# icdm-adteam/MoCoPCI

Measured on AMD Instinct MI355X. Metric: interpolated frames/sec, higher is better.
Workload: dtype f32 (fused MLP layers: fp32 products as 6 bf16-MFMA partials of an exact 3-way split, fp32 accumulate; index paths exact f32)

## Files before the change

### mocopci_amd/csrc/cross.hip

```cpp
#include "common.h"
#include "cross_tile.h"

#ifdef MCP_CROSS_DIAG
__device__ unsigned long long g_cross_diag[8];
#define CROSS_STAMP(slot)                                                                            \
    do {                                                                                             \
        unsigned long long t_;                                                                       \
        __builtin_amdgcn_sched_barrier(0);                                                           \
        asm volatile("s_memtime %0\n\ts_waitcnt lgkmcnt(0)" : "=s"(t_)::"memory");                   \
        __builtin_amdgcn_sched_barrier(0);                                                           \
        if (blockIdx.x == 0 && blockIdx.y == 0 && threadIdx.x == 0) g_cross_diag[slot] += t_ - t_prev; \
        t_prev = t_;                                                                                 \
    } while (0)
#else
#define CROSS_STAMP(slot)
#endif

namespace {

constexpr int MAX_MAPPED_BATCH = 1024;

template <int CTRL>
__device__ __forceinline__ float dppf(float v) {
    return __uint_as_float(mcp_dpp<CTRL>(__float_as_uint(v)));
}
#define MCP_MAX_DPP(dst, src0, src1, CTRL)                                                                              \
    asm("s_nop 1\n\tv_max_f32_dpp %0, %1, %2 " CTRL : "+v"(dst) : "v"(src0), "v"(src1))

__device__ __forceinline__ float scatter_max(const f32x16 &acc, int lane) {
    float v8[8], v4[4], v2[2];
#pragma unroll
    for (int r = 0; r < 8; ++r) {
        const auto sw = __builtin_amdgcn_permlane16_swap(__float_as_uint(acc[r]), __float_as_uint(acc[r + 8]), false, false);
        const float a = __uint_as_float(sw[0]), b = __uint_as_float(sw[1]);
        asm("v_max_f32 %0, %1, %2" : "=v"(v8[r]) : "v"(a), "v"(b));
    }
#pragma unroll
    for (int r = 0; r < 4; ++r) {
        float d = v8[r + 4];
        MCP_MAX_DPP(d, v8[r], v8[r], "row_ror:8 row_mask:0xf bank_mask:0x3");
        MCP_MAX_DPP(d, v8[r + 4], d, "row_ror:8 row_mask:0xf bank_mask:0xc");
        v4[r] = d;
    }
#pragma unroll
    for (int r = 0; r < 2; ++r) {
        float d = v4[r + 2];
        MCP_MAX_DPP(d, v4[r], v4[r], "row_half_mirror row_mask:0xf bank_mask:0x5");
        MCP_MAX_DPP(d, v4[r + 2], d, "row_half_mirror row_mask:0xf bank_mask:0xa");
        v2[r] = d;
    }
    const bool b1 = (lane & 2) != 0;
    float keep = b1 ? v2[1] : v2[0];
    const float send = b1 ? v2[0] : v2[1];
    MCP_MAX_DPP(keep, send, keep, "quad_perm:[2,3,0,1] row_mask:0xf bank_mask:0xf");
    MCP_MAX_DPP(keep, keep, keep, "quad_perm:[1,0,3,2] row_mask:0xf bank_mask:0xf");
    return keep;
}
__device__ __forceinline__ int scatter_reg(int lane) { return ((lane >> 4) & 1) * 8 + ((lane >> 3) & 1) * 4 + ((lane >> 2) & 1) * 2 + ((lane >> 1) & 1); }

template <int D>
__global__ __launch_bounds__(256) void cross_pack_kernel(const float *__restrict__ wpos, const float *__restrict__ bpos,
                                                         const float *__restrict__ wmlp, const float *__restrict__ bmlp,
                                                         float *__restrict__ packed) {
    using L = CrossLds<D>;
    for (int e = blockIdx.x * 256 + threadIdx.x; e < L::FLOATS; e += gridDim.x * 256) {
        float v;
        if (e < L::OFF_POS) continue;
        else if (e < L::OFF_B) {
            const int f = e - L::OFF_POS, lane = f & 63, s = (f >> 6) & 1, t = f >> 7;
            const int row = 32 * t + (lane & 31), c = 2 * s + (lane >> 5);
            v = c < 3 ? wpos[row * 3 + c] : bpos[row];
        } else {
            const int f = e - L::OFF_B, r = f & 15, h = (f >> 4) & 1, t = f >> 5;
            v = bmlp[32 * t + mcp_chan_of(r, h)];
        }
        packed[e] = v;
    }
    mcp_split_weights(reinterpret_cast<uint4 *>(packed + L::OFF_W), wmlp, D, L::T, blockIdx.x * 256 + threadIdx.x, gridDim.x * 256);
}

template <int D>
struct CrossShape {
    static constexpr int NW = D == 128 ? 8 : 4;
    static constexpr int WG_PER_CU = D == 64 ? 3 : 1;
    static constexpr int GRID = D == 64 ? 768 : 256;
};

template <int D, int SPLIT>
__global__ __launch_bounds__(64 * CrossShape<D>::NW, CrossShape<D>::WG_PER_CU) void cross_kernel(long long total, int n1, int n2, const float *__restrict__ xyz1,
                                                           const float *__restrict__ xyz2, const float *__restrict__ points1,
                                                           const float *__restrict__ points2, const int *__restrict__ idx,
                                                           const int *__restrict__ idx2, const int *__restrict__ bmap, int shared,
                                                           const float *__restrict__ packed, float *__restrict__ out) {
    using L = CrossLds<D>;
    constexpr int T = L::T;
    constexpr int WAVES = CrossShape<D>::NW;
    constexpr int TO = T / SPLIT;
    constexpr int WH = L::W_FLOATS / SPLIT, SMALL = L::POS_FLOATS + L::B_FLOATS;
    extern __shared__ __attribute__((aligned(16))) float lds[];
    const int tid = threadIdx.x, split = blockIdx.y;
    static_assert(WH % 4 == 0 && SMALL % 4 == 0, "LDS image is copied as float4");
    for (int e = tid; e < WH / 4; e += 64 * WAVES)
        reinterpret_cast<float4 *>(lds)[e] = reinterpret_cast<const float4 *>(packed + L::OFF_W + (size_t)split * WH)[e];
    for (int e = tid; e < SMALL / 4; e += 64 * WAVES)
        reinterpret_cast<float4 *>(lds + WH)[e] = reinterpret_cast<const float4 *>(packed + L::OFF_POS)[e];
    if (bmap) {
        const int nb = (int)(total / n1);
        for (int e = tid; e < nb; e += 64 * WAVES) reinterpret_cast<int *>(lds + WH + SMALL + WAVES * D)[e] = bmap[e];
    }
    __syncthreads();

    const int lane = tid & 63, wave = tid >> 6, h = lane >> 5, col = lane & 31;
    const float *lpos = lds + WH, *lbias = lds + WH + L::POS_FLOATS;
    float *row1_lds = lds + WH + SMALL + wave * D;
    const int *bmap_lds = reinterpret_cast<const int *>(lds + WH + SMALL + WAVES * D);

#ifndef MCP_NO_XCD_MAP
    const bool by_xcd = gridDim.x >= 8 && (gridDim.x & 7) == 0;
#else
    const bool by_xcd = false;
#endif
    const long long chunk = by_xcd ? (total + 7) / 8 : total;
    const long long stride = (long long)(by_xcd ? gridDim.x >> 3 : gridDim.x) * WAVES;
    const long long limit = by_xcd ? min(total, ((long long)(blockIdx.x & 7) + 1) * chunk) : total;
    long long p = by_xcd ? (long long)(blockIdx.x & 7) * chunk + (long long)(blockIdx.x >> 3) * WAVES + wave : (long long)blockIdx.x * WAVES + wave;
    float q2x = 0.f, q2y = 0.f, q2z = 0.f, p1x = 0.f, p1y = 0.f, p1z = 0.f;
    float4 r1 = make_float4(0.f, 0.f, 0.f, 0.f);
    float4 rg[T][4];
    auto mapped = [&](int bb, int flag) -> long long { return (bmap && (shared & flag)) ? (long long)bmap_lds[bb] : (long long)bb; };
    struct Pos { int bb, off; };
    const int stride_b = (int)(stride / n1), stride_o = (int)(stride % n1);
    auto advance = [&](Pos q) {
        q.bb += stride_b;
        q.off += stride_o;
        if (q.off >= n1) { q.off -= n1; ++q.bb; }
        return q;
    };
    auto fetch = [&](long long pp, Pos q, int id) {
        const float *q2 = xyz2 + ((long long)q.bb * n2 + id) * 3;
        q2x = q2[0]; q2y = q2[1]; q2z = q2[2];
        p1x = xyz1[pp * 3 + 0]; p1y = xyz1[pp * 3 + 1]; p1z = xyz1[pp * 3 + 2];
        const float4 *row2 = reinterpret_cast<const float4 *>(points2 + (mapped(q.bb, 2) * n2 + id) * D);
        const float4 *row1 = reinterpret_cast<const float4 *>(points1 + (mapped(q.bb, 1) * n1 + q.off) * D);
        r1 = row1[lane < D / 4 ? lane : 0];
#pragma unroll
        for (int t = 0; t < T; ++t)
#pragma unroll
            for (int g = 0; g < 4; ++g) rg[t][g] = row2[(32 * t + 8 * g + 4 * h) >> 2];
    };
    auto nbr = [&](long long pp, Pos q) { return cross_nbr(idx, idx2, pp, [&] { return mapped(q.bb, 4) * n1 + q.off; }, col); };
    long long pn = p + stride;
    Pos qp{(int)(p / n1), (int)(p % n1)};
    Pos qn = advance(qp), qnn = advance(qn);
    int idn = 0;
    if (p < limit) {
        fetch(p, qp, nbr(p, qp));
        if (pn < limit) idn = nbr(pn, qn);
    }
#ifdef MCP_CROSS_DIAG
    unsigned long long t_prev = 0;
    CROSS_STAMP(7);
#endif
    for (; p < limit; p = pn, pn += stride) {
        CROSS_STAMP(0);
        McpSplit3 xs[2 * T];
        const float in0 = h ? q2y - p1y : q2x - p1x, in1 = h ? 1.0f : q2z - p1z;
        if (lane < D / 4) reinterpret_cast<float4 *>(row1_lds)[lane] = r1;
        __builtin_amdgcn_wave_barrier();
#pragma unroll
        for (int t = 0; t < T; ++t) {
            f32x16 acc;
#pragma unroll
            for (int g = 0; g < 4; ++g) {
                const float4 a = reinterpret_cast<const float4 *>(row1_lds)[(32 * t + 8 * g + 4 * h) >> 2];
                acc[4 * g + 0] = a.x; acc[4 * g + 1] = a.y; acc[4 * g + 2] = a.z; acc[4 * g + 3] = a.w;
            }
            acc = __builtin_amdgcn_mfma_f32_32x32x2f32(lpos[(t * 2 + 0) * 64 + lane], in0, acc, 0, 0, 0);
            acc = __builtin_amdgcn_mfma_f32_32x32x2f32(lpos[(t * 2 + 1) * 64 + lane], in1, acc, 0, 0, 0);
#pragma unroll
            for (int g = 0; g < 4; ++g) {
                acc[4 * g + 0] = leaky(acc[4 * g + 0] + rg[t][g].x);
                acc[4 * g + 1] = leaky(acc[4 * g + 1] + rg[t][g].y);
                acc[4 * g + 2] = leaky(acc[4 * g + 2] + rg[t][g].z);
                acc[4 * g + 3] = leaky(acc[4 * g + 3] + rg[t][g].w);
            }
            xs[2 * t + 0] = mcp_split_kstep(acc, 0);
            xs[2 * t + 1] = mcp_split_kstep(acc, 1);
        }
        __builtin_amdgcn_wave_barrier();
        CROSS_STAMP(1);
        if (pn < limit) {
            fetch(pn, qn, idn);
            if (pn + stride < limit) idn = nbr(pn + stride, qnn);
        }
        qn = qnn;
        qnn = advance(qnn);
        CROSS_STAMP(2);
#pragma unroll 1
        for (int tl = 0; tl < TO; ++tl) {
            const int t = TO * split + tl;
            f32x16 acc;
#pragma unroll
            for (int r = 0; r < 16; ++r) acc[r] = lbias[(t * 2 + h) * 16 + r];
            acc = mcp_tile_split<2 * T>(reinterpret_cast<const uint4 *>(lds) + (size_t)tl * (2 * T) * 3 * 64 + lane, xs, acc);
            CROSS_STAMP(3);
            const float m = leaky(scatter_max(acc, lane));
            if ((lane & 1) == 0) out[p * D + 32 * t + mcp_chan_of(scatter_reg(lane), h)] = m;
            CROSS_STAMP(4);
        }
    }
}

__global__ __launch_bounds__(64 * X256_WAVES, 1) void cross256_stream_kernel(long long total, int n1, int n2, const float *__restrict__ xyz1,
                                                                          const float *__restrict__ xyz2, const float *__restrict__ points1,
                                                                          const float *__restrict__ points2, const int *__restrict__ idx,
                                                                          const int *__restrict__ idx2, const int *__restrict__ bmap, int shared,
                                                                          const float *__restrict__ packed, float *__restrict__ out) {
    using L = CrossLds<256>;
    constexpr int D = 256, T = X256_T, WAVES = X256_WAVES, SMALL = L::POS_FLOATS + L::B_FLOATS;
    extern __shared__ __attribute__((aligned(16))) float lds[];
    uint4 *wbuf = reinterpret_cast<uint4 *>(lds);
    float *small = lds + 2 * X256_TILE_U4 * 4;
    float *row1_all = small + SMALL;
    int *bmap_lds = reinterpret_cast<int *>(row1_all + WAVES * D);
    const int tid = threadIdx.x, lane = tid & 63, wave = tid >> 6, h = lane >> 5, col = lane & 31;
    const uint4 *wimg = reinterpret_cast<const uint4 *>(packed + L::OFF_W);
    for (int e = tid; e < SMALL / 4; e += 64 * WAVES) reinterpret_cast<float4 *>(small)[e] = reinterpret_cast<const float4 *>(packed + L::OFF_POS)[e];
    if (bmap) {
        const int nb = (int)(total / n1);
        for (int e = tid; e < nb; e += 64 * WAVES) bmap_lds[e] = bmap[e];
    }
    for (int e = tid; e < X256_TILE_U4; e += 64 * WAVES) wbuf[e] = wimg[e];
    __syncthreads();
    const float *lpos = small, *lbias = small + L::POS_FLOATS;
    float *row1_lds = row1_all + wave * D;
    auto mapped = [&](int bb, int flag) -> long long { return (bmap && (shared & flag)) ? (long long)bmap_lds[bb] : (long long)bb; };

    const long long per_round = (long long)gridDim.x * WAVES;
    const long long first = (long long)blockIdx.x * WAVES;
    const int rounds = first < total ? (int)((total - first + per_round - 1) / per_round) : 0;
    int cur = 0;
    for (int g = 0; g < rounds; ++g) {
        const long long pw = first + (long long)g * per_round + wave;
        const bool live = pw < total;
        const long long p = live ? pw : total - 1;
        const int bb = (int)(p / n1), off = (int)(p - (long long)bb * n1);
        int id;
        if (!idx2) {
            id = idx[p * KNB + col];
        } else {
            const long long ps = mapped(bb, 4) * n1 + off;
            id = col >= 16 ? idx2[p * 16 + col - 16] : idx[ps * 16 + col];
        }
        const float *q2 = xyz2 + ((long long)bb * n2 + id) * 3;
        const float dx = q2[0] - xyz1[p * 3 + 0], dy = q2[1] - xyz1[p * 3 + 1], dz = q2[2] - xyz1[p * 3 + 2];
        const float in0 = h ? dy : dx, in1 = h ? 1.0f : dz;
        const float4 *row2 = reinterpret_cast<const float4 *>(points2 + (mapped(bb, 2) * n2 + id) * D);
        const float4 *row1 = reinterpret_cast<const float4 *>(points1 + (mapped(bb, 1) * n1 + off) * D);
        reinterpret_cast<float4 *>(row1_lds)[lane] = row1[lane];
        __builtin_amdgcn_wave_barrier();
        McpSplit3 xs[2 * T];
#pragma unroll
        for (int t = 0; t < T; ++t) {
            f32x16 acc;
            float4 rg[4];
#pragma unroll
            for (int gq = 0; gq < 4; ++gq) {
                const float4 a = reinterpret_cast<const float4 *>(row1_lds)[(32 * t + 8 * gq + 4 * h) >> 2];
                rg[gq] = row2[(32 * t + 8 * gq + 4 * h) >> 2];
                acc[4 * gq + 0] = a.x; acc[4 * gq + 1] = a.y; acc[4 * gq + 2] = a.z; acc[4 * gq + 3] = a.w;
            }
            acc = __builtin_amdgcn_mfma_f32_32x32x2f32(lpos[(t * 2 + 0) * 64 + lane], in0, acc, 0, 0, 0);
            acc = __builtin_amdgcn_mfma_f32_32x32x2f32(lpos[(t * 2 + 1) * 64 + lane], in1, acc, 0, 0, 0);
#pragma unroll
            for (int gq = 0; gq < 4; ++gq) {
                acc[4 * gq + 0] = leaky(acc[4 * gq + 0] + rg[gq].x);
                acc[4 * gq + 1] = leaky(acc[4 * gq + 1] + rg[gq].y);
                acc[4 * gq + 2] = leaky(acc[4 * gq + 2] + rg[gq].z);
                acc[4 * gq + 3] = leaky(acc[4 * gq + 3] + rg[gq].w);
            }
            xs[2 * t + 0] = mcp_split_kstep(acc, 0);
            xs[2 * t + 1] = mcp_split_kstep(acc, 1);
        }
        __builtin_amdgcn_wave_barrier();
#pragma unroll 1
        for (int t = 0; t < T; ++t) {
            const bool more = t + 1 < T || g + 1 < rounds;
            const uint4 *nsrc = wimg + (size_t)((t + 1) & (T - 1)) * X256_TILE_U4 + tid;
            uint4 nx[X256_TILE_U4 / (64 * X256_WAVES)];
#pragma unroll
            for (int i = 0; i < X256_TILE_U4 / (64 * WAVES); ++i) nx[i] = more ? nsrc[i * 64 * WAVES] : make_uint4(0u, 0u, 0u, 0u);
            f32x16 acc;
#pragma unroll
            for (int r = 0; r < 16; ++r) acc[r] = lbias[(t * 2 + h) * 16 + r];
            acc = mcp_tile_split<2 * T>(wbuf + (size_t)cur * X256_TILE_U4 + lane, xs, acc);
            const float m = leaky(scatter_max(acc, lane));
            if (live && (lane & 1) == 0) out[p * D + 32 * t + mcp_chan_of(scatter_reg(lane), h)] = m;
            uint4 *ndst = wbuf + (size_t)(cur ^ 1) * X256_TILE_U4 + tid;
#pragma unroll
            for (int i = 0; i < X256_TILE_U4 / (64 * WAVES); ++i) ndst[i * 64 * WAVES] = nx[i];
            __syncthreads();
            cur ^= 1;
        }
    }
}

int launch_cross256(long long total, int n1, int n2, const float *xyz1, const float *xyz2, const float *points1, const float *points2, const int *idx,
                    const int *idx2, const int *bmap, int shared, const float *packed, float *out, hipStream_t s) {
    const size_t lds = (size_t)(X256_LDS_FLOATS + (bmap ? MAX_MAPPED_BATCH : 0)) * sizeof(float);
    if (const int rc = mcp_allow_lds<cross256_stream_kernel>()) return rc;
    const long long want = (total + X256_WAVES - 1) / X256_WAVES;
    const unsigned grid = (unsigned)max(1LL, min(want, 256LL));
    hipLaunchKernelGGL(cross256_stream_kernel, dim3(grid), dim3(64 * X256_WAVES), lds, s, total, n1, n2, xyz1, xyz2, points1, points2, idx, idx2, bmap, shared,
                       packed, out);
    return mcp_launch_status();
}

template <int D, int SPLIT>
int launch_cross(long long total, int n1, int n2, const float *xyz1, const float *xyz2, const float *points1, const float *points2,
                 const int *idx, const int *idx2, const int *bmap, int shared, const float *packed, float *out, hipStream_t s) {
    using L = CrossLds<D>;
    constexpr int WAVES = CrossShape<D>::NW;
    const size_t lds = (L::W_FLOATS / SPLIT + L::POS_FLOATS + L::B_FLOATS + WAVES * D + (bmap ? MAX_MAPPED_BATCH : 0)) * sizeof(float);
    constexpr auto kern = cross_kernel<D, SPLIT>;
    if (const int rc = mcp_allow_lds<kern>()) return rc;
    const long long want = (total + WAVES * 8 - 1) / (WAVES * 8);
    const unsigned grid = (unsigned)max(1LL, min(want, (long long)(CrossShape<D>::GRID / SPLIT)));
    hipLaunchKernelGGL(kern, dim3(grid, SPLIT), dim3(64 * WAVES), lds, s, total, n1, n2, xyz1, xyz2, points1, points2, idx, idx2, bmap, shared, packed, out);
    return mcp_launch_status();
}

}

MCP_EXPORT int mcp_cross_packed_floats(int d) {
    return d == 64 ? CrossLds<64>::FLOATS : d == 128 ? CrossLds<128>::FLOATS : d == 256 ? CrossLds<256>::FLOATS : 0;
}

MCP_EXPORT int mcp_cross_pack(int d, const float *wpos, const float *bpos, const float *wmlp, const float *bmlp, float *packed,
                              mcp_stream_t stream) {
    MCP_CHECK_ARGS(wpos && bpos && wmlp && bmlp && packed);
    if (d != 64 && d != 128 && d != 256) return MCP_ERR_UNSUPPORTED;
    if (((uintptr_t)packed) & 15) return MCP_ERR_BAD_ARG;
    hipStream_t s = (hipStream_t)stream;
    if (d == 64) hipLaunchKernelGGL(cross_pack_kernel<64>, dim3(16), dim3(256), 0, s, wpos, bpos, wmlp, bmlp, packed);
    else if (d == 128) hipLaunchKernelGGL(cross_pack_kernel<128>, dim3(64), dim3(256), 0, s, wpos, bpos, wmlp, bmlp, packed);
    else hipLaunchKernelGGL(cross_pack_kernel<256>, dim3(256), dim3(256), 0, s, wpos, bpos, wmlp, bmlp, packed);
    return mcp_launch_status();
}

MCP_EXPORT int mcp_cross_volume(int b, int n1, int n2, int d, int k, const float *xyz1, const float *xyz2, const float *points1,
                                const float *points2, const int *idx, const int *idx2, const int *bmap, int shared, const float *packed, float *out,
                                mcp_stream_t stream) {
    MCP_CHECK_ARGS(b > 0 && n1 > 0 && n2 > 0 && xyz1 && xyz2 && points1 && points2 && idx && packed && out);
    if (k != KNB || (d != 64 && d != 128 && d != 256)) return MCP_ERR_UNSUPPORTED;
    if ((((uintptr_t)points1) | ((uintptr_t)points2) | ((uintptr_t)out) | ((uintptr_t)packed)) & 15) return MCP_ERR_BAD_ARG;
    if (bmap && b > MAX_MAPPED_BATCH) return MCP_ERR_UNSUPPORTED;
    hipStream_t s = (hipStream_t)stream;
    const long long total = (long long)b * n1;
    mcp_prof_begin(MCP_KERNEL_CROSS, s);
    const int rc = d == 64    ? launch_cross<64, 1>(total, n1, n2, xyz1, xyz2, points1, points2, idx, idx2, bmap, shared, packed, out, s)
                   : d == 128 ? launch_cross<128, 1>(total, n1, n2, xyz1, xyz2, points1, points2, idx, idx2, bmap, shared, packed, out, s)
                              : launch_cross256(total, n1, n2, xyz1, xyz2, points1, points2, idx, idx2, bmap, shared, packed, out, s);
    mcp_prof_end(MCP_KERNEL_CROSS, s);
    return rc;
}

#ifdef MCP_CROSS_DIAG
MCP_EXPORT int mcp_cross_diag_read(unsigned long long *out8) {
    hipError_t e = hipMemcpyFromSymbol(out8, HIP_SYMBOL(g_cross_diag), sizeof(unsigned long long) * 8);
    unsigned long long z[8] = {0};
    (void)hipMemcpyToSymbol(HIP_SYMBOL(g_cross_diag), z, sizeof(z));
    return (int)e;
}
#endif
```

Before: 3669.

## Interleave layer-1 split work into layer-2 k-steps for D=128 cross kernel

For D=128 (by default), the cross kernel switches from a tile-major loop to a k-step-major schedule. The next tile's layer-1 MFMAs, leaky activation and 3-way bf16 split are interleaved as fill work inside the layer-2 MFMA k-steps, and the weight fragments for the next step are software-prefetched. The intent is to hide VALU split and activation work and LDS latency behind the MFMA pipeline, and to keep fewer split registers live. The cost is more accumulator registers (TO accumulators at once), more complex code, and possible register pressure or spills. The diagnostic timers also move to per-thread slot accumulation.

```diff
diff --git a/mocopci_amd/csrc/cross.hip b/mocopci_amd/csrc/cross.hip
--- a/mocopci_amd/csrc/cross.hip
+++ b/mocopci_amd/csrc/cross.hip
@@ -1,3 +1,4 @@
+#include <utility>
 #include "common.h"
 #include "cross_tile.h"
 
@@ -9,7 +10,7 @@
         __builtin_amdgcn_sched_barrier(0);                                                           \
         asm volatile("s_memtime %0\n\ts_waitcnt lgkmcnt(0)" : "=s"(t_)::"memory");                   \
         __builtin_amdgcn_sched_barrier(0);                                                           \
-        if (blockIdx.x == 0 && blockIdx.y == 0 && threadIdx.x == 0) g_cross_diag[slot] += t_ - t_prev; \
+        t_slot[slot] += t_ - t_prev;                                                                 \
         t_prev = t_;                                                                                 \
     } while (0)
 #else
@@ -84,7 +85,46 @@
     static constexpr int NW = D == 128 ? 8 : 4;
     static constexpr int WG_PER_CU = D == 64 ? 3 : 1;
     static constexpr int GRID = D == 64 ? 768 : 256;
+#if defined(MCP_CROSS_TILE_MAJOR)
+    static constexpr bool KSTEP_MAJOR = false;
+#elif defined(MCP_CROSS_KSTEP_MAJOR_64)
+    static constexpr bool KSTEP_MAJOR = true;
+#else
+    static constexpr bool KSTEP_MAJOR = D == 128;
+#endif
 };
+
+__device__ __forceinline__ void x0_pair(f32x16 &a, const float4 *rg, int i) {
+    const float4 g = rg[i >> 1];
+    a[2 * i + 0] = leaky(a[2 * i + 0] + ((i & 1) ? g.z : g.x));
+    a[2 * i + 1] = leaky(a[2 * i + 1] + ((i & 1) ? g.w : g.y));
+}
+__device__ __forceinline__ void split_pair(const f32x16 &a, int i, McpSplit3 *xs) {
+    const float v0 = a[2 * i], v1 = a[2 * i + 1];
+    const float r0 = v0 - __uint_as_float(mcp_top16(v0)), r1 = v1 - __uint_as_float(mcp_top16(v1));
+    const float s0 = r0 - __uint_as_float(mcp_top16(r0)), s1 = r1 - __uint_as_float(mcp_top16(r1));
+    const uint32_t d1 = mcp_pack_hi(v0, v1), d2 = mcp_pack_hi(r0, r1), d3 = mcp_pack_hi(s0, s1);
+    McpSplit3 &o = xs[i >> 2];
+    switch (i & 3) {
+        case 0: o.p1.x = d1; o.p2.x = d2; o.p3.x = d3; break;
+        case 1: o.p1.y = d1; o.p2.y = d2; o.p3.y = d3; break;
+        case 2: o.p1.z = d1; o.p2.z = d2; o.p3.z = d3; break;
+        default: o.p1.w = d1; o.p2.w = d2; o.p3.w = d3; break;
+    }
+}
+constexpr int NF_X0_PAIR = 6, NF_SPLIT_PAIR = 11;
+
+struct CrossFill { int l0, l1, s0, s1; };
+template <class F, int... I>
+__device__ __forceinline__ void cross_static_for_(F &&f, std::integer_sequence<int, I...>) { (f(std::integral_constant<int, I>{}), ...); }
+template <int N, class F>
+__device__ __forceinline__ void cross_static_for(F &&f) { cross_static_for_(f, std::make_integer_sequence<int, N>{}); }
+template <int NK>
+__device__ __forceinline__ constexpr CrossFill cross_fill(int j) {
+    if (NK == 4) return CrossFill{4 + j, 5 + j, 2 * j, 2 * j + 2};
+    if (j >= 3) return CrossFill{j, j + 1, j, j + 1};
+    return j == 0 ? CrossFill{0, 0, 0, 0} : j == 1 ? CrossFill{0, 2, 0, 1} : CrossFill{2, 3, 1, 3};
+}
 
 template <int D, int SPLIT>
 __global__ __launch_bounds__(64 * CrossShape<D>::NW, CrossShape<D>::WG_PER_CU) void cross_kernel(long long total, int n1, int n2, const float *__restrict__ xyz1,
@@ -148,21 +188,139 @@
 #pragma unroll
             for (int g = 0; g < 4; ++g) rg[t][g] = row2[(32 * t + 8 * g + 4 * h) >> 2];
     };
+    const int *bmap_any = bmap ? bmap_lds : reinterpret_cast<const int *>(lds);
+    auto mapped_sel = [&](int bb, int flag) -> long long {
+        const bool use = bmap && (shared & flag);
+        const int m = bmap_any[use ? bb : 0];
+        return use ? (long long)m : (long long)bb;
+    };
+    auto fetch_head = [&](long long pp, Pos q, int id) {
+        const float *q2 = xyz2 + ((long long)q.bb * n2 + id) * 3;
+        q2x = q2[0]; q2y = q2[1]; q2z = q2[2];
+        p1x = xyz1[pp * 3 + 0]; p1y = xyz1[pp * 3 + 1]; p1z = xyz1[pp * 3 + 2];
+        const float4 *row1 = reinterpret_cast<const float4 *>(points1 + (mapped_sel(q.bb, 1) * n1 + q.off) * D);
+        r1 = row1[lane < D / 4 ? lane : 0];
+    };
+    auto row2_of = [&](Pos q, int id) { return reinterpret_cast<const float4 *>(points2 + (mapped_sel(q.bb, 2) * n2 + id) * D); };
+    auto nbr_sel = [&](long long pp, int bb, int off) {
+        const long long ps = mapped_sel(bb, 4) * n1 + off;
+        const bool two = idx2 != nullptr, second = two && col >= 16;
+        const int *list = second ? idx2 : idx;
+        const long long row = two && !second ? ps : pp;
+        const long long at16 = row * 16 + (col & 15), at32 = row * KNB + col;
+        return list[two ? at16 : at32];
+    };
     auto nbr = [&](long long pp, Pos q) { return cross_nbr(idx, idx2, pp, [&] { return mapped(q.bb, 4) * n1 + q.off; }, col); };
     long long pn = p + stride;
     Pos qp{(int)(p / n1), (int)(p % n1)};
     Pos qn = advance(qp), qnn = advance(qn);
     int idn = 0;
+    [[maybe_unused]] int idc = 0;
+    [[maybe_unused]] Pos qc = qp;
     if (p < limit) {
-        fetch(p, qp, nbr(p, qp));
+        idc = nbr(p, qp);
+        fetch(p, qp, idc);
         if (pn < limit) idn = nbr(pn, qn);
     }
 #ifdef MCP_CROSS_DIAG
-    unsigned long long t_prev = 0;
+    unsigned long long t_prev = 0, t_slot[8] = {0, 0, 0, 0, 0, 0, 0, 0};
     CROSS_STAMP(7);
 #endif
     for (; p < limit; p = pn, pn += stride) {
         CROSS_STAMP(0);
+      if constexpr (CrossShape<D>::KSTEP_MAJOR) {
+        static_assert(SPLIT == 1 && (T == 2 || T == 4), "cross_fill's batches are laid out for 4 or 8 k-steps per block");
+        constexpr int NK = 2 * TO;
+        const float in0 = h ? q2y - p1y : q2x - p1x, in1 = h ? 1.0f : q2z - p1z;
+        if (lane < D / 4) reinterpret_cast<float4 *>(row1_lds)[lane] = r1;
+        __builtin_amdgcn_wave_barrier();
+        auto layer1_begin = [&](int t) {
+            f32x16 a;
+#pragma unroll
+            for (int g = 0; g < 4; ++g) {
+                const float4 v = reinterpret_cast<const float4 *>(row1_lds)[(32 * t + 8 * g + 4 * h) >> 2];
+                a[4 * g + 0] = v.x; a[4 * g + 1] = v.y; a[4 * g + 2] = v.z; a[4 * g + 3] = v.w;
+            }
+            a = __builtin_amdgcn_mfma_f32_32x32x2f32(lpos[(t * 2 + 0) * 64 + lane], in0, a, 0, 0, 0);
+            return __builtin_amdgcn_mfma_f32_32x32x2f32(lpos[(t * 2 + 1) * 64 + lane], in1, a, 0, 0, 0);
+        };
+        f32x16 xb[2];
+        McpSplit3 xs[2][2];
+        constexpr bool EARLY1 = NK == 4;
+        xb[0] = layer1_begin(0);
+        if constexpr (EARLY1) xb[1] = layer1_begin(1);
+        if constexpr (T == 2) __builtin_amdgcn_wave_barrier();
+#pragma unroll
+        for (int i = 0; i < 8; ++i) {
+            x0_pair(xb[0], rg[0], i);
+            split_pair(xb[0], i, xs[0]);
+        }
+        if constexpr (NK == 4) {
+#pragma unroll
+            for (int i = 0; i < 4; ++i) x0_pair(xb[1], rg[1], i);
+        }
+        __builtin_amdgcn_sched_barrier(0);
+        CROSS_STAMP(1);
+        const bool more = pn < limit;
+        idc = more ? idn : idc;
+        qc = more ? qn : qc;
+        const float4 *row2n = row2_of(qc, idc);
+        fetch_head(more ? pn : p, qc, idc);
+        const bool more2 = pn + stride < limit;
+        idn = nbr_sel(more2 ? pn + stride : more ? pn : p, more2 ? qnn.bb : qc.bb, more2 ? qnn.off : qc.off);
+#pragma unroll
+        for (int g = 0; g < 4; ++g) rg[0][g] = row2n[(8 * g + 4 * h) >> 2];
+        f32x16 acc[TO];
+#pragma unroll
+        for (int tl = 0; tl < TO; ++tl)
+#pragma unroll
+            for (int r = 0; r < 16; ++r) acc[tl][r] = lbias[((TO * split + tl) * 2 + h) * 16 + r];
+        const uint4 *wl = reinterpret_cast<const uint4 *>(lds) + lane;
+        uint4 w1 = wl[0], w2 = wl[64], w3 = wl[128];
+        cross_static_for<T>([&](auto tc) {
+            constexpr int t = decltype(tc)::value;
+            if constexpr ((t >= 1 || !EARLY1) && t + 1 < T) {
+                xb[(t + 1) & 1] = layer1_begin(t + 1);
+                if constexpr (t + 2 == T) __builtin_amdgcn_wave_barrier();
+            }
+            cross_static_for<NK>([&](auto jc) {
+                constexpr int j = decltype(jc)::value, tl = j % TO, ks = j / TO;
+                uint4 n1 = w1, n2 = w2, n3 = w3;
+                if constexpr (t * NK + j + 1 < T * NK) {
+                    constexpr int jn = (j + 1) % NK, tn = t + (j + 1) / NK;
+                    const uint4 *nx = wl + (size_t)((jn % TO) * 2 * T + 2 * tn + jn / TO) * 3 * 64;
+                    n1 = nx[0]; n2 = nx[64]; n3 = nx[128];
+                }
+                const McpSplit3 &x = xs[t & 1][ks];
+                if constexpr (t + 1 < T) {
+                    constexpr CrossFill f = cross_fill<NK>(j);
+                    constexpr int nf = NF_X0_PAIR * (f.l1 - f.l0) + NF_SPLIT_PAIR * (f.s1 - f.s0), u = t + 1;
+                    acc[tl] = mcp_kstep_fill<nf>(w1, w2, w3, x, acc[tl], [&] {
+#pragma unroll
+                        for (int i = f.l0; i < f.l1; ++i) x0_pair(xb[u & 1], rg[u], i);
+#pragma unroll
+                        for (int i = f.s0; i < f.s1; ++i) split_pair(xb[u & 1], i, xs[u & 1]);
+                    });
+                } else {
+                    acc[tl] = mcp_kstep_fill<0>(w1, w2, w3, x, acc[tl], [] {});
+                }
+                w1 = n1; w2 = n2; w3 = n3;
+            });
+            CROSS_STAMP(2 + t);
+            if constexpr (t + 1 < T) {
+#pragma unroll
+                for (int g = 0; g < 4; ++g) rg[t + 1][g] = row2n[(32 * (t + 1) + 8 * g + 4 * h) >> 2];
+            }
+        });
+#pragma unroll
+        for (int tl = 0; tl < TO; ++tl) {
+            const float m = leaky(scatter_max(acc[tl], lane));
+            if ((lane & 1) == 0) out[p * D + 32 * (TO * split + tl) + mcp_chan_of(scatter_reg(lane), h)] = m;
+        }
+        CROSS_STAMP(6);
+        qn = qnn;
+        qnn = advance(qnn);
+      } else {
         McpSplit3 xs[2 * T];
         const float in0 = h ? q2y - p1y : q2x - p1x, in1 = h ? 1.0f : q2z - p1z;
         if (lane < D / 4) reinterpret_cast<float4 *>(row1_lds)[lane] = r1;
@@ -188,14 +346,13 @@
             xs[2 * t + 1] = mcp_split_kstep(acc, 1);
         }
         __builtin_amdgcn_wave_barrier();
-        CROSS_STAMP(1);
         if (pn < limit) {
             fetch(pn, qn, idn);
             if (pn + stride < limit) idn = nbr(pn + stride, qnn);
         }
         qn = qnn;
         qnn = advance(qnn);
-        CROSS_STAMP(2);
+        CROSS_STAMP(1);
 #pragma unroll 1
         for (int tl = 0; tl < TO; ++tl) {
             const int t = TO * split + tl;
@@ -203,12 +360,17 @@
 #pragma unroll
             for (int r = 0; r < 16; ++r) acc[r] = lbias[(t * 2 + h) * 16 + r];
             acc = mcp_tile_split<2 * T>(reinterpret_cast<const uint4 *>(lds) + (size_t)tl * (2 * T) * 3 * 64 + lane, xs, acc);
-            CROSS_STAMP(3);
+            CROSS_STAMP(2);
             const float m = leaky(scatter_max(acc, lane));
             if ((lane & 1) == 0) out[p * D + 32 * t + mcp_chan_of(scatter_reg(lane), h)] = m;
-            CROSS_STAMP(4);
-        }
-    }
+            CROSS_STAMP(6);
+        }
+      }
+    }
+#ifdef MCP_CROSS_DIAG
+    if (blockIdx.x == 0 && blockIdx.y == 0 && threadIdx.x == 0)
+        for (int s = 0; s < 7; ++s) g_cross_diag[s] += t_slot[s];
+#endif
 }
 
 __global__ __launch_bounds__(64 * X256_WAVES, 1) void cross256_stream_kernel(long long total, int n1, int n2, const float *__restrict__ xyz1,
```

Result: no change. 3679, median of 5 (+0.3%).
